# 0xPabloxx/3d-pointcloud-orientation-estimation

Hardware: AMD Instinct MI355X
Metric: clouds/sec fwd+bwd, pointnet_pp_vonMises N=1024 (higher is better)
Workload: dtype f32; 1 GPU; configs[1]: models/pointnet_pp_vonMises.py single-peak KL, N=1024, batch=32 per GPU, fwd+loss+bwd+allreduce+Adam, random-init weights (seed 42), device-side centre sampling; per_gpu_batch=32, global_batch=32, points=1024, parallelism=single, launch=hipGraph(fwd+loss+bwd) + eager all-reduce/Adam (the update clears the gradients)

## Files before the change

3d-pointcloud-orientation-estimation_amd/csrc/dw_kernels.hip:

```cpp
#include "gemm_smallm.h"
#include "launch.h"
#include "split_prims.h"

namespace pnpp {

template <int DZMODE, int A2MODE, int CT, int KT>
__global__ void __launch_bounds__(256)
dw_kernel(const AOperand dz, const AOperand a2, int M, int Nc, int Kp, int tilesC, int tilesK, int rows_per_split,
          int kp_pad, float *__restrict__ slab, int policy) {
    constexpr int U = 4;
    const int lane = threadIdx.x & 63, l31 = lane & 31, lh = lane >> 5;
    const int gw = blockIdx.x * 4 + (threadIdx.x >> 6);
    const int tiles = tilesC * tilesK;
    const int tile = gw % tiles, split = gw / tiles;
    const int r0 = min(M, split * rows_per_split);
    const int r1 = min(M, r0 + rows_per_split);
    const int c0 = (tile % tilesC) * 32 * CT, k0 = (tile / tilesC) * 32 * KT;

    ChanConst cc[CT], ck[KT];
#pragma unroll
    for (int i = 0; i < CT; ++i) cc[i] = load_chan_const<DZMODE>(dz, c0 + i * 32 + l31, Nc);
#pragma unroll
    for (int j = 0; j < KT; ++j) ck[j] = load_chan_const<A2MODE>(a2, k0 + j * 32 + l31, Kp);

    f32x16 acc[CT][KT];
#pragma unroll
    for (int i = 0; i < CT; ++i)
#pragma unroll
        for (int j = 0; j < KT; ++j)
#pragma unroll
            for (int r = 0; r < 16; ++r) acc[i][j][r] = 0.f;

// ... 171 lines not shown
        for (int e = 0; e < 4; ++e) d1[e] += (double)s1[e], d2[e] += (double)s2[e];
    }
    if (slab == nullptr) return;
#pragma unroll
    for (int e = 0; e < 4; ++e) {
        gred[(rl * 2 + 0) * C + c4 + e] = d1[e];
        gred[(rl * 2 + 1) * C + c4 + e] = d2[e];
    }
    __syncthreads();
    for (int f = threadIdx.x; f < 2 * C; f += 256) {
        const int which = f / C, c = f - which * C;
        double t = 0.0;
        for (int w = 0; w < RPP; ++w) t += gred[(w * 2 + which) * C + c];
        sp_store(slab + ((size_t)blockIdx.x * 2 + which) * C + c, t, (policy & ST_STAT_SLABS) != 0);
    }
}

bool delayed_layer0_ok(int C) {
    return C >= 32 && C <= 512 && (C & (C - 1)) == 0;
}

int launch_gather_rel_stats(const float *P, const AOperand &geo, const float *W0, int ldw, int M, int C, float *z,
                            double *slab, int *nslab, hipStream_t st) {
    PNPP_REQUIRE(delayed_layer0_ok(C) && geo.mode == A_GATHER, PNPP_ERR_ARG, "gather_rel_stats: unsupported width %d", C);
    const int rpp = 256 / (C / 4);
    int rpb = 64;
    while (rpb < 4 * rpp || cdiv(M, rpb) > kMaxStatBlocks) rpb *= 2;
    const int grid = cdiv(M, rpb);
    if (nslab) *nslab = grid;
    ProfScope ps(st, "gather_rel_stats_kernel M=%d C=%d grid=%d", M, C, grid);
    hipLaunchKernelGGL(gather_rel_stats_kernel, dim3(grid), dim3(256), (size_t)rpp * 2 * C * sizeof(double), st, P, geo.xyz,
                       geo.new_xyz, geo.idx, W0, ldw, geo.N, geo.S, geo.K, M, C, rpb, z, slab, store_policy());
    PNPP_CHECK_LAUNCH("gather_rel_stats");
    return PNPP_OK;
}

constexpr int SCW = 8;
constexpr int SCWIN = 1024;
template <int NCH>
__global__ void __launch_bounds__(SCW * 64)
scatter_dz_kernel(const AOperand dz, const AOperand geo, int Mc, int C, int total, float *__restrict__ G,
                  float *__restrict__ wslab) {
    constexpr int UB = NCH == 1 ? 8 : 4;
    __shared__ int hl[SCW][SCWIN];
    __shared__ float wred[SCW][NCH * 128][3];
    const int lane = threadIdx.x & 63, wv = threadIdx.x >> 6;
    const int N = geo.N;
    const int dst = min(blockIdx.x * SCW + wv, total - 1);
    const bool live = blockIdx.x * SCW + wv < total;
    const int b = dst / N, n = dst - b * N;
    const int32_t *ib = geo.idx + (size_t)b * Mc;
    const size_t row0 = (size_t)b * Mc;
    const float px = geo.xyz[(size_t)dst * 3], py = geo.xyz[(size_t)dst * 3 + 1], pz = geo.xyz[(size_t)dst * 3 + 2];
    const float *cb = geo.new_xyz + (size_t)b * geo.S * 3;
    float2 cg[NCH], cmu[NCH], cis[NCH], c1[NCH], c2[NCH], acc[NCH], ax[NCH], ay[NCH], az[NCH];
    int cc[NCH];
#pragma unroll
    for (int j = 0; j < NCH; ++j) {
        cc[j] = min(j * 128 + 2 * lane, C - 2);
        cg[j] = make_float2(1.f, 1.f);
        cmu[j] = cis[j] = c1[j] = c2[j] = acc[j] = ax[j] = ay[j] = az[j] = make_float2(0.f, 0.f);
        if (dz.mode == A_DZ) {
            const float *p = dz.cst + cc[j];
            cg[j] = *reinterpret_cast<const float2 *>(p), cmu[j] = *reinterpret_cast<const float2 *>(p + dz.C);
            cis[j] = *reinterpret_cast<const float2 *>(p + 2 * dz.C), c1[j] = *reinterpret_cast<const float2 *>(p + 3 * dz.C);
            c2[j] = *reinterpret_cast<const float2 *>(p + 4 * dz.C);
// ... 253 lines not shown
    if (!(M > 32 && M <= 4096 && cdiv(M, 32) <= kMaxStatBlocks && dz.mode == A_PLAIN && (dz.lda & 3) == 0 && ((uintptr_t)dz.a & 15) == 0))
        return false;
    if (!(Nc >= 128 && Kp >= 128 && Kd % 4 == 0 && !Win.trans && (E.mode == E_STORE || E.mode == E_MASK_STATS))) return false;
    if (!(a2.mode == A_PLAIN || a2.mode == A_BNRELU || a2.mode == A_CONCAT)) return false;
    if (a2.mode != A_CONCAT && ((a2.lda & 3) != 0 || ((uintptr_t)a2.a & 15) != 0)) return false;
    if (kp_pad != cdiv(Kp, 64) * 64 || nsplit < 1) return false;
    BOperand W = Win;
    if (W.rows <= 0 || W.rows > Kd) W.rows = Kd;
    const int g1x = cdiv(Nout, 32), g1y = cdiv(M, 32), g1 = g1x * g1y;
    const int tc = cdiv(Nc, 128), tk = cdiv(Kp, 128);
    int rps = cdiv(M, nsplit);
    rps = (rps + 7) & ~7;
    const dim3 grid(g1 + tc * tk * nsplit);
    if (nslab) *nslab = g1y;
    ProfScope ps(st, "da_dw_kernel<E%d,A%d> M=%d | dA N=%d K=%d grid=%d | dW N=%d K=%d split=%d grid=%d", E.mode, a2.mode, M, Nout, Kd, g1,
                 Nc, Kp, nsplit, tc * tk * nsplit);
#define PNPP_DADW(EM, AM) \
    hipLaunchKernelGGL((da_dw_kernel<EM, AM>), grid, dim3(256), 0, st, dz, W, M, Nout, Kd, E, g1x, g1, a2, Nc, Kp, tc, tk, rps, kp_pad, slab)
    if (E.mode == E_STORE) {
        if (a2.mode == A_PLAIN) PNPP_DADW(E_STORE, A_PLAIN);
        else if (a2.mode == A_BNRELU) PNPP_DADW(E_STORE, A_BNRELU);
        else PNPP_DADW(E_STORE, A_CONCAT);
    } else {
        if (a2.mode == A_PLAIN) PNPP_DADW(E_MASK_STATS, A_PLAIN);
        else if (a2.mode == A_BNRELU) PNPP_DADW(E_MASK_STATS, A_BNRELU);
        else PNPP_DADW(E_MASK_STATS, A_CONCAT);
    }
#undef PNPP_DADW
    check_launch("da_dw", rc);
    return true;
}

}
```

3d-pointcloud-orientation-estimation_amd/csrc/kernels.h:

```cpp
#pragma once
#include "common.h"

namespace pnpp {

int launch_knn(const float *new_xyz, const float *xyz, int B, int S, int N, int k, int32_t *idx, hipStream_t st,
               const int32_t *lengths = nullptr);
int launch_knn_centres(const float *xyz, const int32_t *centre, int B, int S, int N, int k, int32_t *idx, float *out_a,
                       float *out_b, hipStream_t st, const int32_t *lengths = nullptr);
int launch_knn_pair(const float *xyz, int B, int N, const int32_t *centre1, int S1, int k1, int32_t *idx1, float *a1, float *b1,
                    const int32_t *centre2, int S2, int k2, int32_t *idx2, float *a2, float *b2, double *mom, hipStream_t st,
                    const int32_t *lengths = nullptr);
int knn_pair_moment_partials(int B, int S1, int N);
size_t knn_pair_moment_doubles(int B, int S1, int N);
int launch_gather_centres(const float *xyz, const int32_t *centre, int B, int N, int S, float *out_a, float *out_b, hipStream_t st);
int launch_scatter_rows_bwd(const float *dout, const int32_t *idx, int B, int N, int C, int M, float *dpoints, hipStream_t st);

enum AMode {
    A_PLAIN = 0,
    A_BNRELU = 1,
    A_GATHER = 2,
    A_CONCAT = 3,
    A_DZ = 4,
    A_DZ_POOL = 5
};
// ... 75 lines not shown
struct PoolTail {
    const float *pool_ext = nullptr;
    float *pool_out = nullptr;
    int32_t *pool_arg = nullptr;
    float *origin_a = nullptr, *origin_b = nullptr;
    int G = 0, norigin = 0;
};
struct DzSide { const AOperand *dz = nullptr; int M = 0; float *out = nullptr; };
struct SlabReduceArgs {
    const float *slab;
    int nsplit, Nc, kp_pad, Kvalid, perm_D;
    float *out;
    int ldo;
};

int launch_gemm(const AOperand &A, const BOperand &B, int M, int Nout, int Kd, const Epilogue &E, int *nslab,
                hipStream_t st, int *dw_slabs = nullptr);
bool mid_tiles_on();
bool try_launch_ws(const AOperand &A, const BOperand &B, int M, int Nout, int Kd, const Epilogue &E, int *nslab, hipStream_t st, int *rc,
                   int *dw_slabs);

int matmul_precision();
void set_matmul_precision(int bf16);
bool try_launch_ws_bf16(const AOperand &A, const BOperand &B, int M, int Nout, int Kd, const Epilogue &E, int *nslab, hipStream_t st,
                        int *rc, int *dw_slabs);

int launch_dw(const AOperand &dz, int Nc, const AOperand &a2, int Kp, int M, float *slab, int nsplit, int kp_pad,
              hipStream_t st);
int launch_dz_materialize(const AOperand &dz, int M, int C, float *out, hipStream_t st);
void dw_plan(int M, int Nc, int Kp, int *nsplit, int *kp_pad);
bool delayed_layer0_ok(int C);
int launch_gather_rel_stats(const float *P, const AOperand &geo, const float *W0, int ldw, int M, int C, float *z,
                            double *slab, int *nslab, hipStream_t st);
int scatter_dz_splits(int rows);
int launch_scatter_dz(const AOperand &dz, const AOperand &geo, int B, int Mc, int C, float *G, float *wslab, hipStream_t st);
int dw_xyz_splits(int M);
int launch_dw_xyz(const AOperand &dz, int Nc, const AOperand &a2, int M, float *slab, hipStream_t st);
bool try_launch_fc_dx_dw(const float *dz, const float *w, const float *x, int M, int N, int K, float *dx, float *dw, hipStream_t st,
                         int *rc);
bool try_launch_da_dw(const AOperand &dz, const BOperand &W, int M, int Nout, int Kd, const Epilogue &E, int *nslab, const AOperand &a2,
                      int Kp, float *slab, int *nsplit, int *kp_pad, hipStream_t st, int *rc, float *dw_direct = nullptr, int dw_ld = 0);
bool try_launch_mid_gemm(const AOperand &A, const BOperand &B, int M, int Nout, int Kd, const Epilogue &E, int *nslab, hipStream_t st,
                         int *rc);
bool mid_gemm_pools(const AOperand &A, int M, int Nout, int Kd);
bool try_launch_wsf(const AOperand &A, const BOperand &B, int M, int Nout, int Kd, const Epilogue &E, int *nslab, hipStream_t st, int *rc);
bool wsf_applies(const AOperand &A, const BOperand &B, int M, int Nout, int Kd, const Epilogue &E);
int split_products();
void set_split_products(int on);
int store_policy();
void set_store_policy(int mask);
bool try_launch_wsf3(const AOperand &A, const BOperand &B, int M, int Nout, int Kd, const Epilogue &E, int *nslab, hipStream_t st, int *rc);
bool try_launch_wsd3(const AOperand &A, const BOperand &B, int M, int Nout, int Kd, const Epilogue &E, int *nslab, hipStream_t st, int *rc,
                     int *dw_slabs);
int wsd3_timeouts();
bool try_launch_wsp(const AOperand &A, const BOperand &B, int M, int Nout, int Kd, const Epilogue &E, int *nslab, hipStream_t st, int *rc,
                    int *dw_slabs);
bool try_launch_wsq(const AOperand &A, const BOperand &B, int M, int Nout, int Kd, const Epilogue &E, int *nslab, hipStream_t st, int *rc,
                    int *dw_slabs);
bool try_launch_wsx(const AOperand &dz, const BOperand &W, int M, int C1, int C0, const AOperand &geo, const float *W0, int ldw0,
                    const float *scale0, const float *shift0, float *dwslab, double *stat, int *workers_out, hipStream_t st, int *rc);
size_t wsx_stat_doubles();
bool xyz0_applies(int M, int D, int K, int group_all, int L, const int *C);
size_t xyz0_moment_doubles();
int launch_rel_moments(const AOperand &geo, int M, double *mom, int *nmom, hipStream_t st);
int launch_wsf0(const AOperand &geo, int M, const BOperand &W0, const double *mom, int nmom, const BnLayer &bn0, const BnHyper &h,
                const BOperand &W1, const Epilogue &E, int *nslab, hipStream_t st);
// ... 62 lines not shown
```

3d-pointcloud-orientation-estimation_amd/csrc/sa_api.hip:

```cpp
#include "launch.h"

namespace pnpp {

struct SaGeom {
    int M, G, maxC;
    int Cin[PNPP_MAX_LAYERS];
    int Kd[PNPP_MAX_LAYERS];
};

static int sa_geom(const pnpp_sa_desc *d, SaGeom *g) {
    PNPP_REQUIRE(d, PNPP_ERR_ARG, "sa: null descriptor");
    PNPP_REQUIRE(d->B > 0 && d->N > 0 && d->S > 0 && d->K > 0 && d->D >= 0, PNPP_ERR_ARG,
                 "sa: bad geometry B=%d N=%d S=%d K=%d D=%d", d->B, d->N, d->S, d->K, d->D);
    PNPP_REQUIRE(d->L >= 1 && d->L <= PNPP_MAX_LAYERS, PNPP_ERR_ARG, "sa: unsupported layer count %d", d->L);
    if (d->group_all) PNPP_REQUIRE(d->S == 1 && d->K == d->N, PNPP_ERR_ARG, "sa: group_all needs S == 1 and K == N");
    PNPP_REQUIRE((long long)d->B * d->S * d->K < (1ll << 31), PNPP_ERR_ARG, "sa: B*S*K overflows int32");
    g->M = d->B * d->S * d->K;
    g->G = d->B * d->S;
    g->maxC = 0;
    for (int l = 0; l < d->L; ++l) {
        PNPP_REQUIRE(d->C[l] > 0 && d->C[l] % 32 == 0, PNPP_ERR_ARG,
                     "sa: mlp channel %d (=%d) must be a positive multiple of 32 for the MFMA path", l, d->C[l]);
        g->maxC = d->C[l] > g->maxC ? d->C[l] : g->maxC;
        g->Cin[l] = l == 0 ? d->D + 3 : d->C[l - 1];
// ... 190 lines not shown
    sa_level_bind(L, a->saved, a->scratch, a->xyz, a->points, a->conv_w, a->bn_w, st);
    L->hyper = BnHyper{d->momentum, d->eps, d->training ? 1 : 0};
    return PNPP_OK;
}

static int sa_fwd_group(const SaLevel &L, const pnpp_sa_fwd_args *a) {
    const pnpp_sa_desc *d = L.d;
    const SaSaved &sv = L.sv;
    if (d->group_all) return PNPP_OK;
    PNPP_REQUIRE(d->S <= d->N, PNPP_ERR_RANGE, "sa_forward: npoint=%d > N=%d", d->S, d->N);
    if (a->neighbour_idx == sv.idx) return PNPP_OK;
    if (!a->neighbour_idx)
        return launch_knn_centres(a->xyz, a->centre_idx, d->B, d->S, d->N, d->K, sv.idx, a->new_xyz, sv.new_xyz, L.st);
    PNPP_TRY(launch_gather_centres(a->xyz, a->centre_idx, d->B, d->N, d->S, a->new_xyz, sv.new_xyz, L.st));
    hipError_t e = hipMemcpyAsync(sv.idx, a->neighbour_idx, (size_t)L.g.M * sizeof(int32_t), hipMemcpyDeviceToDevice, L.st);
    PNPP_REQUIRE(e == hipSuccess, PNPP_ERR_LAUNCH, "sa_forward: neighbour copy failed: %s", hipGetErrorString(e));
    return PNPP_OK;
}

static int sa_fwd_finalize(const SaLevel &L, int l, int nslab, const PoolTail *tail = nullptr) {
    StatsView V;
    if (L.d->training) PNPP_TRY(stats_exchange(L.sc.slab, nslab, L.d->C[l], L.count(), L.st, &V));
    return launch_bn_finalize_fwd(V, L.count(), L.bn[l], L.hyper, L.st, tail);
}

static int sa_fwd_gemm(const SaLevel &L, int l, const AOperand &A, const BOperand &W, const Epilogue &E, const double *mom, int nmom, int *ns) {
    if (L.xyz0 && l == 1)
        return launch_wsf0(L.layer0_operand(), L.g.M, L.weight(0, 0), mom, nmom, L.bn[0], L.hyper, L.weight(1, 0), E, ns, L.st);
    return launch_gemm(A, W, L.g.M, L.d->C[l], L.g.Kd[l], E, ns, L.st);
}

static int sa_fwd_delayed0(const SaLevel &L, const AOperand &geo) {
    const pnpp_sa_desc *d = L.d;
    AOperand F;
    F.a = L.points, F.lda = d->D;
    BOperand Wf = L.w0_features();
    Wf.trans = 1, Wf.rows = d->D;
    int nslab = 0;
    PNPP_TRY(launch_gemm(F, Wf, d->B * d->N, d->C[0], d->D, store_to(L.sc.src, d->C[0]), nullptr, L.st));
    PNPP_TRY(launch_gather_rel_stats(L.sc.src, geo, L.conv_w[0], L.g.Cin[0], L.g.M, d->C[0], L.sv.z[0], d->training ? L.sc.slab : nullptr,
                                     &nslab, L.st));
    return sa_fwd_finalize(L, 0, nslab);
}

static int sa_forward_impl(const pnpp_sa_desc *d, const pnpp_sa_fwd_args *a, hipStream_t st) {
    SaLevel L;
    PNPP_TRY(sa_level_fwd(d, a, st, &L));
    const SaGeom &g = L.g;
    const SaSaved &sv = L.sv;
    const SaScratch &sc = L.sc;
    PNPP_TRY(sa_fwd_group(L, a));
    const int Lm = d->L - 1;
    bool pooled = false;
    int nmom = 0;
    const double *mom = sc.mom;
    for (int l = 0; l < d->L; ++l) {
        if (L.xyz0 && l == 0) {
            if (!d->training) PNPP_TRY(sa_fwd_finalize(L, 0, 0));
            else if (a->neighbour_idx == sv.idx && L.pair_moments) mom = sv.mom, nmom = knn_pair_moment_partials(d->B, d->S, d->N);
            else PNPP_TRY(launch_rel_moments(L.layer0_operand(), g.M, sc.mom, &nmom, st));
            continue;
        }
        const AOperand A = L.input_of(l);
        if (l == 0 && L.delayed) {
            PNPP_TRY(sa_fwd_delayed0(L, A));
            continue;
// ... 331 lines not shown
```

3d-pointcloud-orientation-estimation_amd/csrc/split_prims.h:

```cpp
#pragma once
#include <type_traits>

#include "common.h"

namespace pnpp {
namespace {

typedef __bf16 bf16x8 __attribute__((ext_vector_type(8)));
typedef __bf16 bf16x2v __attribute__((ext_vector_type(2)));
typedef float f32x2v __attribute__((ext_vector_type(2)));
typedef short s16x4 __attribute__((ext_vector_type(4)));

__device__ __forceinline__ unsigned sp_pk(float lo, float hi) {
    const f32x2v v = {lo, hi};
    return __builtin_bit_cast(unsigned, __builtin_convertvector(v, bf16x2v));
}
__device__ __forceinline__ float sp_lo(unsigned p) { return __uint_as_float(p << 16); }
__device__ __forceinline__ float sp_hi(unsigned p) { return __uint_as_float(p & 0xffff0000u); }
__device__ __forceinline__ void sp_split2(float v0, float v1, unsigned &h, unsigned &m, unsigned &l) {
    h = sp_pk(v0, v1);
    float r0 = v0 - sp_lo(h), r1 = v1 - sp_hi(h);
    m = sp_pk(r0, r1);
    r0 -= sp_lo(m), r1 -= sp_hi(m);
    l = sp_pk(r0, r1);
// ... 16 lines not shown
    const s16x4 v = __builtin_amdgcn_ds_read_tr16_b64_v4i16((__attribute__((address_space(3))) s16x4 *)(p));
    return __builtin_bit_cast(uint2, v);
}
__device__ __forceinline__ constexpr int sp_swz_row(int r) { return (((r >> 1) & 1) << 2) | ((r >> 2) & 3); }

__device__ __forceinline__ __amdgpu_buffer_rsrc_t sp_buf_rsrc_n(const void *base, unsigned records) {
    return __builtin_amdgcn_make_buffer_rsrc(const_cast<void *>(base), (short)0, records, 0x00020000);
}
__device__ __forceinline__ __amdgpu_buffer_rsrc_t sp_buf_rsrc(const void *base) { return sp_buf_rsrc_n(base, 0xfffffffe); }
__device__ __forceinline__ __amdgpu_buffer_rsrc_t sp_buf_rsrc_null(const void *base) { return sp_buf_rsrc_n(base, 0); }
__device__ __forceinline__ f32x4 sp_buf_load4(__amdgpu_buffer_rsrc_t r, unsigned lane_off, unsigned s_off) {
    return __builtin_bit_cast(f32x4, __builtin_amdgcn_raw_buffer_load_b128(r, (int)lane_off, (int)s_off, 0));
}
__device__ __forceinline__ float sp_buf_load1(__amdgpu_buffer_rsrc_t r, unsigned lane_off, unsigned s_off) {
    return __builtin_bit_cast(float, __builtin_amdgcn_raw_buffer_load_b32(r, (int)lane_off, (int)s_off, 0));
}

template <typename F>
__device__ __forceinline__ void sp_with_policy(bool wt, F &&f) {
    if (wt) f(std::true_type{});
    else f(std::false_type{});
}
template <typename T>
__device__ __forceinline__ void sp_store(T *p, T v, bool wt) {
    static_assert(sizeof(T) == 4 || sizeof(T) == 8, "one dword or two per lane");
    typedef __attribute__((address_space(1))) T gT;
    if (wt) __hip_atomic_store((gT *)p, v, __ATOMIC_RELAXED, __HIP_MEMORY_SCOPE_AGENT);
    else *p = v;
}
__device__ __forceinline__ void sp_buf_store1(float v, __amdgpu_buffer_rsrc_t r, unsigned lane_off, unsigned s_off, bool wt) {
    if (wt) __builtin_amdgcn_raw_buffer_store_b32(__builtin_bit_cast(unsigned, v), r, (int)lane_off, (int)s_off, 16);
    else __builtin_amdgcn_raw_buffer_store_b32(__builtin_bit_cast(unsigned, v), r, (int)lane_off, (int)s_off, 0);
}

}
}
```

3d-pointcloud-orientation-estimation_amd/pnpp_hip/_lib.py:

```python
from __future__ import annotations

import ctypes as C
import os

HERE = os.path.dirname(os.path.abspath(__file__))
LIB_PATH = os.path.join(HERE, "libpnpp_hip.so")

PNPP_MAX_LAYERS = 4
PNPP_OK, PNPP_ERR_ARG, PNPP_ERR_RANGE, PNPP_ERR_LAUNCH, PNPP_ERR_WORKSPACE = 0, -1, -2, -3, -4
NORM_NONE, NORM_BATCH, NORM_LAYER = 0, 1, 2

_fp = C.c_void_p


class SaDesc(C.Structure):
    _fields_ = [("B", C.c_int), ("N", C.c_int), ("S", C.c_int), ("K", C.c_int), ("D", C.c_int), ("L", C.c_int),
                ("C", C.c_int * PNPP_MAX_LAYERS), ("group_all", C.c_int), ("training", C.c_int),
                ("eps", C.c_float), ("momentum", C.c_float)]


_PL = _fp * PNPP_MAX_LAYERS


class SaFwdArgs(C.Structure):
# ... 210 lines not shown
    "pnpp_orient_eval": (_i, [_fp, _fp, _fp, _i, _i, _fp, _fp, _fp, _fp, _i, _fp, _i, _fp, _fp, C.c_int64, _fp, _fp, _fp, _fp]),
    "pnpp_log_softmax": (_i, [_fp, _i, _i, _fp, _fp]),
    "pnpp_log_softmax_bwd": (_i, [_fp, _fp, _i, _i, _fp, _fp]),
    "pnpp_linear_log_softmax": (_i, [_fp, _fp, _fp, _i, _i, _i, _fp, _fp]),
    "pnpp_nll_loss": (_i, [_fp, _fp, _i, _i, _fp, _fp, _i, _fp]),
    "pnpp_nll_loss_bwd": (_i, [_fp, _fp, _i, _i, _fp, _fp]),
    "pnpp_l2_normalize": (_i, [_fp, _i, _i, _f, _fp, _fp]),
    "pnpp_l2_normalize_bwd": (_i, [_fp, _fp, _i, _i, _f, _fp, _fp]),
    "pnpp_mse": (_i, [_fp, _fp, _sz, _fp, _fp, _fp]),
    "pnpp_mse_rows": (_i, [_fp, _fp, _i, _i, _fp, _fp, _fp]),
    "pnpp_orth_loss": (_i, [_fp, _fp, _i, _i, _fp, _fp, _fp, _fp]),
    "pnpp_proj_probs": (_i, [_fp, _fp, _i, _i, _fp, _fp]),
    "pnpp_proj_probs_bwd": (_i, [_fp, _fp, _fp, _i, _i, _fp, _fp]),
    "pnpp_linear_smallk": (_i, [_fp, _fp, _fp, _i, _i, _i, _fp, _fp]),
    "pnpp_attention_fwd": (_i, [_fp, _i, _i, _i, _i, _i, _fp, _f, _fp, _fp, _fp]),
    "pnpp_attention_dropout_mask": (_i, [_u64, _u64, _i, _i, _i, _f, _fp, _fp, _fp]),
    "pnpp_attention_dropout_mask_dev": (_i, [_u64, _fp, _u64, _i, _i, _i, _f, _fp, _fp, _fp]),
    "pnpp_add_layernorm": (_i, [_fp, _fp, _fp, _fp, _i, _i, _f, _fp, _fp]),
    "pnpp_mean_points": (_i, [_fp, _i, _i, _i, _fp, _fp]),
    "pnpp_linear_smallk_bwd_scratch_bytes": (_sz, [_i, _i]),
    "pnpp_linear_smallk_bwd": (_i, [_fp, _fp, _i, _i, _i, _fp, _fp, _fp, _fp]),
    "pnpp_attention_bwd": (_i, [_fp, _fp, _fp, _fp, _i, _i, _i, _i, _i, _fp, _fp, _f, _fp, _fp, _fp]),
    "pnpp_add_layernorm_bwd_scratch_bytes": (_sz, [_i, _i]),
    "pnpp_add_layernorm_bwd": (_i, [_fp, _fp, _fp, _fp, _i, _i, _f, _fp, _fp, _fp, _fp]),
    "pnpp_mean_points_bwd": (_i, [_fp, _i, _i, _i, _fp, _fp]),
    "pnpp_set_matmul_precision": (_i, [_i]),
    "pnpp_set_stats_exchange": (_i, [STATS_EXCHANGE_FN, C.c_void_p, C.c_void_p, _sz]),
    "pnpp_stats_exchange_enabled": (_i, []),
    "pnpp_get_matmul_precision": (_i, []),
    "pnpp_set_split_products": (_i, [_i]),
    "pnpp_get_split_products": (_i, []),
    "pnpp_set_store_policy": (_i, [_i]),
    "pnpp_get_store_policy": (_i, []),
    "pnpp_adam_step": (_i, [_fp, _fp, _fp, _fp, _sz, _i, _f, _f, _f, _f, _f, _fp]),
    "pnpp_adam_step_zero": (_i, [_fp, _fp, _fp, _fp, _sz, _i, _f, _f, _f, _f, _f, _fp]),
    "pnpp_adam_step_dev": (_i, [_fp, _fp, _fp, _fp, _sz, _fp, _f, _f, _f, _f, _f, _i, _fp]),
    "pnpp_adam_step_clip": (_i, [_fp, _fp, _fp, _fp, _sz, _i, _f, _f, _f, _f, _f, _fp, _f, _i, _fp]),
    "pnpp_adam_step_dev_clip": (_i, [_fp, _fp, _fp, _fp, _sz, _fp, _f, _f, _f, _f, _f, _fp, _f, _i, _fp]),
    "pnpp_sumsq": (_i, [_fp, _sz, _fp, _fp, _sz, _fp]),
    "pnpp_adamw_step": (_i, [C.POINTER(OptimDesc), _fp, _fp, _fp, _fp, _fp, _sz, _fp, _fp, _fp]),
    "pnpp_lr_factor": (_i, [C.POINTER(OptimDesc), _u64, C.POINTER(C.c_double)]),
    "pnpp_pn_pool_saved_bytes": (_sz, [C.POINTER(PnPoolDesc)]),
    "pnpp_pn_pool_scratch_bytes": (_sz, [C.POINTER(PnPoolDesc)]),
    "pnpp_pn_pool_forward": (_i, [C.POINTER(PnPoolDesc), C.POINTER(PnPoolFwdArgs), _fp]),
    "pnpp_pn_pool_backward": (_i, [C.POINTER(PnPoolDesc), C.POINTER(PnPoolBwdArgs), _fp]),
    "pnpp_pn_pool_saved_route": (_fp, [C.POINTER(PnPoolDesc), _fp]),
    "pnpp_pn_pool_saved_zsel": (_fp, [C.POINTER(PnPoolDesc), _fp]),
    "pnpp_pn_pool_saved_ypre": (_fp, [C.POINTER(PnPoolDesc), _fp]),
    "pnpp_fc_recompute_output": (_i, [C.POINTER(FcDesc), _fp, _fp, _fp, _fp]),
    "pnpp_pn_transform": (_i, [_fp, C.c_int64, C.c_int64, C.c_int64, _fp, _i, _i, _i, _i, _i, _fp, _fp]),
    "pnpp_pn_transform_bwd": (_i, [_fp, C.c_int64, C.c_int64, C.c_int64, _fp, _fp, _i, _i, _i, _i, _i, _fp, _fp, _fp]),
    "pnpp_pn_regularizer": (_i, [_fp, _i, _i, _fp, _fp, _fp]),
    "pnpp_pn_regularizer_bwd": (_i, [_fp, _fp, _fp, _i, _i, _fp, _fp]),
    "pnpp_pn_add_identity": (_i, [_fp, _i, _i, _fp, _fp]),
    "pnpp_pn_concat": (_i, [_fp, _fp, _i, _i, _i, _i, _fp, _fp]),
    "pnpp_pn_concat_bwd": (_i, [_fp, _i, _i, _i, _i, _fp, _fp, _fp]),
    "pnpp_pn_bn_relu": (_i, [_fp, _i, _i, _fp, _fp, _fp, _fp, _fp, _i, _f, _f, _fp, _fp, _fp, _fp]),
    "pnpp_pn_bn_relu_bwd": (_i, [_fp, _fp, _fp, _i, _i, _fp, _fp, _fp, _i, _fp, _fp, _fp, _fp]),
    "pnpp_pn_offsets": (_i, [_fp, _i, _i, _fp, _fp, _fp]),
    "pnpp_pn_pool_saved_bytes_ragged": (_sz, [C.POINTER(PnPoolDesc), _i]),
    "pnpp_pn_pool_scratch_bytes_ragged": (_sz, [C.POINTER(PnPoolDesc), _i]),
    "pnpp_pn_pool_forward_ragged": (_i, [C.POINTER(PnPoolDesc), C.POINTER(PnPoolFwdArgs), _fp, _i, _fp]),
    "pnpp_pn_pool_backward_ragged": (_i, [C.POINTER(PnPoolDesc), C.POINTER(PnPoolBwdArgs), _fp, _i, _fp]),
    "pnpp_pn_transform_ragged": (_i, [_fp, _i, C.c_int64, C.c_int64, C.c_int64, _fp, _fp, _i, _i, _i, _i, _i, _fp, _fp]),
    "pnpp_pn_transform_bwd_ragged": (_i, [_fp, _i, C.c_int64, C.c_int64, C.c_int64, _fp, _fp, _fp, _i, _i, _i, _i, _i, _fp, _fp, _fp]),
    "pnpp_pn_concat_ragged": (_i, [_fp, _fp, _i, _fp, _i, _i, _i, _i, _fp, _fp]),
# ... 44 lines not shown
```

3d-pointcloud-orientation-estimation_amd/pnpp_hip/ops.py:

```python
from __future__ import annotations

import ctypes as C
import os
from typing import Optional, Sequence, Tuple

import torch

from . import _lib as L
from .lengths import fps_starts, packed_lengths, ragged_lengths


def _stream() -> int:
    return torch.cuda.current_stream().cuda_stream


def _need_gpu(t: torch.Tensor, name: str) -> None:
    if not isinstance(t, torch.Tensor):
        raise TypeError(f"{name} must be a torch.Tensor")
    if not t.is_cuda:
        raise RuntimeError(f"{name} is on '{t.device}': the pnpp HIP operators run on an AMD GPU only "
                           "(no CPU fallback exists in this package)")


def _f32(t: torch.Tensor, name: str) -> torch.Tensor:
# ... 83 lines not shown
        returned.append(fresh)
    return dests, returned


def set_matmul_precision(mode: str) -> None:
    if mode not in ("f32", "bf16"):
        raise ValueError(f"matmul precision must be 'f32' or 'bf16', got {mode!r}")
    L.check(L.lib().pnpp_set_matmul_precision(1 if mode == "bf16" else 0))


def get_matmul_precision() -> str:
    return "bf16" if L.lib().pnpp_get_matmul_precision() else "f32"


def set_float32_products(mode: str) -> None:
    if mode not in ("split", "mfma"):
        raise ValueError(f"float32 products must be 'split' or 'mfma', got {mode!r}")
    L.check(L.lib().pnpp_set_split_products(1 if mode == "split" else 0))


def get_float32_products() -> str:
    return "split" if L.lib().pnpp_get_split_products() else "mfma"


STORE_DW_SLABS, STORE_STAT_SLABS, STORE_STREAMS = 1, 2, 4


def set_store_policy(mask: int) -> None:
    L.check(L.lib().pnpp_set_store_policy(int(mask)))


def get_store_policy() -> int:
    return L.lib().pnpp_get_store_policy()


def square_distance(src: torch.Tensor, dst: torch.Tensor) -> torch.Tensor:
    src, dst = _f32(src, "src"), _f32(dst, "dst")
    B, S, _ = src.shape
    N = dst.shape[1]
    out = torch.empty(B, S, N, device=src.device, dtype=torch.float32)
    L.check(L.lib().pnpp_square_distance(src.data_ptr(), dst.data_ptr(), B, S, N, out.data_ptr(), _stream()))
    return out


def knn(new_xyz: torch.Tensor, xyz: torch.Tensor, k: int, lengths=None) -> torch.Tensor:
    new_xyz, xyz = _f32(new_xyz, "new_xyz"), _f32(xyz, "xyz")
    B, S, _ = new_xyz.shape
    N = xyz.shape[1]
    idx = torch.empty(B, S, k, device=xyz.device, dtype=torch.int32)
    if lengths is not None:
        lengths = ragged_lengths(lengths, B, N, xyz.device, minimum=k)
        L.check(L.lib().pnpp_knn_ragged(new_xyz.data_ptr(), xyz.data_ptr(), B, S, N, lengths.data_ptr(), int(k), idx.data_ptr(), _stream()))
        return idx
    L.check(L.lib().pnpp_knn(new_xyz.data_ptr(), xyz.data_ptr(), B, S, N, int(k), idx.data_ptr(), _stream()))
    return idx


def estimate_normals(xyz: torch.Tensor, k: int, mode: int = L.NORMALS_NONE, ref: Optional[torch.Tensor] = None, lengths=None,
                     stride: int = 3, curvature: bool = False, neighbours: bool = False):
    xyz = _f32(xyz, "xyz")
    if xyz.dim() != 3 or xyz.shape[2] != 3:
        raise ValueError(f"xyz must be (B, N, 3), got {tuple(xyz.shape)}")
    B, N, _ = xyz.shape
    if ref is not None:
        ref = _f32(ref, "ref")
        if tuple(ref.shape) != (B, 3):
# ... 1498 lines not shown
```

include/pnpp_hip.h:

```cpp
#ifndef PNPP_HIP_H
#define PNPP_HIP_H

#include <stddef.h>
#include <stdint.h>

#ifdef __cplusplus
extern "C" {
#endif

typedef enum {
    PNPP_OK = 0,
    PNPP_ERR_ARG = -1,
    PNPP_ERR_RANGE = -2,
    PNPP_ERR_LAUNCH = -3,
    PNPP_ERR_WORKSPACE = -4
} pnpp_status;

const char *pnpp_last_error(void);
int pnpp_abi_version(void);

int pnpp_profile_enable(int on);
int pnpp_profile_report(char *buf_host, size_t buflen);


// ... 224 lines not shown
int pnpp_orth_loss(const float *a, const float *b, int B, int C, float *loss, float *da, float *db, void *stream);
int pnpp_proj_probs(const float *vec, const float *dirs, int B, int D, float *probs, void *stream);
int pnpp_proj_probs_bwd(const float *vec, const float *dirs, const float *dprobs, int B, int D, float *dvec, void *stream);

int pnpp_linear_smallk(const float *x, const float *w, const float *b, int M, int K, int N, float *y, void *stream);
int pnpp_attention_fwd(const float *qkv, int B, int N, int n_valid, int H, int head_dim, const uint32_t *mask, float p,
                       float *out, float *lse, void *stream);
int pnpp_attention_dropout_mask(uint64_t seed, uint64_t stream_id, int B, int N, int H, float p, uint32_t *mask,
                                uint32_t *maskT, void *stream);
int pnpp_attention_dropout_mask_dev(uint64_t seed, uint64_t *stream_id_dev, uint64_t offset, int B, int N, int H, float p,
                                    uint32_t *mask, uint32_t *maskT, void *stream);
int pnpp_add_layernorm(const float *x, const float *r, const float *w, const float *b, int M, int E, float eps, float *y,
                       void *stream);
int pnpp_mean_points(const float *x, int B, int N, int E, float *y, void *stream);
size_t pnpp_linear_smallk_bwd_scratch_bytes(int M, int N);
int pnpp_linear_smallk_bwd(const float *x, const float *dy, int M, int K, int N, float *dw, float *db, void *scratch,
                           void *stream);
int pnpp_attention_bwd(const float *qkv, const float *out, const float *d_out, const float *lse, int B, int N, int n_valid, int H,
                       int head_dim, const uint32_t *mask, const uint32_t *maskT, float p, float *dqkv, float *dsum,
                       void *stream);
size_t pnpp_add_layernorm_bwd_scratch_bytes(int M, int E);
int pnpp_add_layernorm_bwd(const float *x, const float *r, const float *w, const float *dy, int M, int E, float eps,
                           float *du, float *dwb, void *scratch, void *stream);
int pnpp_mean_points_bwd(const float *dy, int B, int N, int E, float *dx, void *stream);

int pnpp_set_matmul_precision(int bf16_operands);
int pnpp_get_matmul_precision(void);

int pnpp_set_split_products(int on);
int pnpp_get_split_products(void);

int pnpp_set_store_policy(int mask);
int pnpp_get_store_policy(void);
int pnpp_debug_wsd3_timeouts(void);

typedef int (*pnpp_stats_exchange_fn)(double *buf, size_t n_doubles, void *stream, void *user);
int pnpp_set_stats_exchange(pnpp_stats_exchange_fn fn, void *user, double *buf, size_t buf_doubles);
int pnpp_stats_exchange_enabled(void);

typedef struct {
    int B, N;
    int K, C;
    int relu;
    int training;
    float eps, momentum;
} pnpp_pn_pool_desc;

typedef struct {
    const float *a;
    const float *w, *b;
    const float *gamma, *beta;
    float *rm, *rv;
    int64_t *nbt;
    float *out;
    void *saved;
    void *scratch;
} pnpp_pn_pool_fwd_args;

typedef struct {
    const float *a, *w, *gamma;
    const float *dout;
    const void *saved;
    void *scratch;
    float *da;
    float *dw, *db, *dgamma, *dbeta;
} pnpp_pn_pool_bwd_args;
// ... 233 lines not shown
```

Baseline: 61050 clouds/s.

## Fuse per-point feature GEMM into delayed layer-0 gather/stats kernel

Adds a fused kernel for the delayed layer-0 path. Each block computes the per-point feature projection P = F·W0 for its batch and channel slice in LDS using MFMA, then gathers neighbour rows, adds the relative-xyz term and accumulates the BN statistics in the same launch. Before, a separate GEMM wrote P to global memory and the stats kernel read it back. The fused form removes one launch and that global round trip, but every share block recomputes P for its whole cloud, and the large LDS footprint may lower occupancy. It is on by default (form=1) when the shape checks pass.

```diff
diff --git a/3d-pointcloud-orientation-estimation_amd/csrc/dw_kernels.hip b/3d-pointcloud-orientation-estimation_amd/csrc/dw_kernels.hip
--- a/3d-pointcloud-orientation-estimation_amd/csrc/dw_kernels.hip
+++ b/3d-pointcloud-orientation-estimation_amd/csrc/dw_kernels.hip
@@ -1,3 +1,5 @@
+#include <algorithm>
+
 #include "gemm_smallm.h"
 #include "launch.h"
 #include "split_prims.h"
@@ -235,6 +237,224 @@
     hipLaunchKernelGGL(gather_rel_stats_kernel, dim3(grid), dim3(256), (size_t)rpp * 2 * C * sizeof(double), st, P, geo.xyz,
                        geo.new_xyz, geo.idx, W0, ldw, geo.N, geo.S, geo.K, M, C, rpb, z, slab, store_policy());
     PNPP_CHECK_LAUNCH("gather_rel_stats");
+    return PNPP_OK;
+}
+
+constexpr int D0_SL = 32;
+constexpr int D0_PP = D0_SL + 4;
+constexpr int D0_ROWS = 256 / (D0_SL / 4);
+constexpr size_t kDelayed0LdsMax = 80 * 1024;
+constexpr int kDelayed0MaxRows = 2048;
+
+static size_t delayed0_lds_bytes(int N, int S, int D, int rps) {
+    const size_t npad = (size_t)cdiv(N, 32) * 32;
+    return sizeof(float) * ((size_t)4 * 32 * APITCH + npad * D0_PP + 4 * (size_t)N + 4 * (size_t)S + (size_t)D0_SL * (D + 1) + (size_t)rps);
+}
+
+static int delayed0_shares(int B, int SK, int C, int *rows_per_share) {
+    int shares = cdiv(256, B * (C / D0_SL));
+    shares = std::min(shares, std::max(1, SK / (4 * D0_ROWS)));
+    shares = std::max(shares, cdiv(SK, kDelayed0MaxRows));
+    const int rps = cdiv(SK, shares);
+    *rows_per_share = rps;
+    return cdiv(SK, rps);
+}
+
+bool delayed0_fused_ok(int B, int N, int S, int K, int D, int C) {
+    if (!(B >= 1 && N >= 1 && S >= 1 && K >= 1 && (long long)S * K < (1 << 24) && D >= 32 && D % 32 == 0 && C % D0_SL == 0 && delayed_layer0_ok(C))) return false;
+    int rps = 0;
+    const int shares = delayed0_shares(B, S * K, C, &rps);
+    return (long long)B * shares <= kMaxStatBlocks && delayed0_lds_bytes(N, S, D, rps) <= kDelayed0LdsMax;
+}
+
+__global__ void __launch_bounds__(256)
+gather_rel_stats_fused_kernel(const float *__restrict__ F, const float *__restrict__ xyz, const float *__restrict__ new_xyz,
+                              const int32_t *__restrict__ idx, const float *__restrict__ W0, int ldw, int B, int N, int S, int K,
+                              int D, int C, int shares, int rps, float *__restrict__ z, double *__restrict__ slab, int policy) {
+    extern __shared__ __attribute__((aligned(16))) float d0lds[];
+    const int tid = threadIdx.x, lane = tid & 63, wave = tid >> 6, l31 = lane & 31, lh = lane >> 5;
+    const int nsl = C / D0_SL, per = nsl * shares;
+    const int q = blockIdx.x >> 3;
+    const int b = (blockIdx.x & 7) + 8 * (q / per);
+    if (b >= B) return;
+    const int sub = q % per, c0 = (sub % nsl) * D0_SL, share = sub / nsl;
+    const int SK = S * K, r0 = share * rps, r1 = min(SK, r0 + rps);
+    const int ntiles = (N + 31) >> 5, nch = D >> 5, WP = D + 1;
+    float *As = d0lds + wave * 32 * APITCH;
+    float *Pl = d0lds + 4 * 32 * APITCH;
+    float4 *Xl = reinterpret_cast<float4 *>(Pl + ntiles * 32 * D0_PP);
+    float4 *Cl = Xl + N;
+    float *Wl = reinterpret_cast<float *>(Cl + S);
+    int *Il = reinterpret_cast<int *>(Wl + D0_SL * WP);
+    const float *Fb = F + (size_t)b * N * D;
+    const int32_t *ib = idx + (size_t)b * SK;
+
+    float4 na[2][4];
+    auto fetch_a = [&](float4(&d)[4], int t, int c) {
+#pragma unroll
+        for (int i = 0; i < 4; ++i) {
+            const int row = min(t * 32 + (lane >> 3) + 8 * i, N - 1);
+            d[i] = *reinterpret_cast<const float4 *>(Fb + (size_t)row * D + c * KC + 4 * (lane & 7));
+        }
+    };
+    auto fetch_a2 = [&](int t) {
+        fetch_a(na[0], t, 0);
+        if (nch > 1) fetch_a(na[1], t, 1);
+    };
+    if (wave < ntiles) fetch_a2(wave);
+    const int rl = tid >> 3, c4 = (tid & 7) * 4;
+    const int i0 = ib[min(r0 + tid, r1 - 1)], i1 = ib[min(r0 + 256 + tid, r1 - 1)];
+    float wx[4], wy[4], wz[4];
+#pragma unroll
+    for (int e = 0; e < 4; ++e) {
+        const float *w = W0 + (size_t)(c0 + c4 + e) * ldw;
+        wx[e] = w[0], wy[e] = w[1], wz[e] = w[2];
+    }
+    const float *xp = xyz + ((size_t)b * N + min(tid, N - 1)) * 3, *cp = new_xyz + ((size_t)b * S + min(tid, S - 1)) * 3;
+    const float x0 = xp[0], x1 = xp[1], x2 = xp[2], q0 = cp[0], q1 = cp[1], q2 = cp[2];
+    {
+        int wr = tid / D, wk = tid - wr * D;
+        const int dq = 256 / D, dm = 256 - dq * D;
+        auto w_batch = [&](auto nb) {
+            float t[nb()];
+            int o[nb()];
+#pragma unroll
+            for (int u = 0; u < nb(); ++u) {
+                t[u] = W0[(size_t)(c0 + wr) * ldw + 3 + wk];
+                o[u] = wr * WP + wk;
+                wr += dq, wk += dm;
+                if (wk >= D) wk -= D, ++wr;
+            }
+#pragma unroll
+            for (int u = 0; u < nb(); ++u) Wl[o[u]] = t[u];
+        };
+        int e0 = 0;
+        for (; e0 + 4096 <= D0_SL * D; e0 += 4096) w_batch(mode_c<16>{});
+        for (; e0 < D0_SL * D; e0 += 1024) w_batch(mode_c<4>{});
+    }
+    if (tid < N) Xl[tid] = make_float4(x0, x1, x2, 0.f);
+    if (tid < S) Cl[tid] = make_float4(q0, q1, q2, 0.f);
+    if (r0 + tid < r1) Il[tid] = i0;
+    if (r0 + 256 + tid < r1) Il[256 + tid] = i1;
+    for (int i = r0 + 512 + tid; i < r1; i += 256) Il[i - r0] = ib[i];
+    for (int i = tid + 256; i < N; i += 256) {
+        const float *x = xyz + ((size_t)b * N + i) * 3;
+        Xl[i] = make_float4(x[0], x[1], x[2], 0.f);
+    }
+    for (int i = tid + 256; i < S; i += 256) {
+        const float *c = new_xyz + ((size_t)b * S + i) * 3;
+        Cl[i] = make_float4(c[0], c[1], c[2], 0.f);
+    }
+    __syncthreads();
+
+    for (int t = wave; t < ntiles; t += 4) {
+        f32x16 acc4[4];
+#pragma unroll
+        for (int i = 0; i < 4; ++i)
+#pragma unroll
+            for (int r = 0; r < 16; ++r) acc4[i][r] = 0.f;
+        if (t != wave) fetch_a2(t);
+        auto chunk = [&](f32x16 &acc, float4(&d)[4], int c) {
+#pragma unroll
+            for (int i = 0; i < 4; ++i) {
+                const int o = ((lane >> 3) + 8 * i) * APITCH + 4 * (lane & 7);
+                As[o] = d[i].x, As[o + 1] = d[i].y, As[o + 2] = d[i].z, As[o + 3] = d[i].w;
+            }
+            if (c + 2 < nch) fetch_a(d, t, c + 2);
+            const float *wk = Wl + l31 * WP + c * KC + lh;
+#pragma unroll
+            for (int s2 = 0; s2 < KC / 2; ++s2)
+                acc = __builtin_amdgcn_mfma_f32_32x32x2f32(As[l31 * APITCH + 2 * s2 + lh], wk[2 * s2], acc, 0, 0, 0);
+        };
+        for (int c = 0; c < nch; c += 4) {
+            chunk(acc4[0], na[0], c);
+            if (c + 1 < nch) chunk(acc4[1], na[1], c + 1);
+            if (c + 2 < nch) chunk(acc4[2], na[0], c + 2);
+            if (c + 3 < nch) chunk(acc4[3], na[1], c + 3);
+        }
+#pragma unroll
+        for (int r = 0; r < 16; ++r)
+            Pl[(t * 32 + (r & 3) + 8 * (r >> 2) + 4 * lh) * D0_PP + l31] = (acc4[0][r] + acc4[1][r]) + (acc4[2][r] + acc4[3][r]);
+    }
+    __syncthreads();
+
+    double d1[4] = {0.0, 0.0, 0.0, 0.0}, d2[4] = {0.0, 0.0, 0.0, 0.0};
+    float *zc = z + (size_t)b * SK * C;
+    const int Ro = 1024 / C, ro = (rl / Ro) * 4 * Ro + rl % Ro;
+    const float rcpK = 1.f / (float)K;
+    const __amdgpu_buffer_rsrc_t zr = sp_buf_rsrc(zc);
+    sp_with_policy((policy & ST_STREAMS) != 0, [&](auto wt) {
+    for (int rb = r0 + ro; rb - ro < r1; rb += 4 * D0_ROWS) {
+        int jc[4];
+#pragma unroll
+        for (int u = 0; u < 4; ++u) jc[u] = Il[min(rb + u * Ro, r1 - 1) - r0];
+        float4 p[4];
+        float rx[4], ry[4], rz[4], ok[4];
+#pragma unroll
+        for (int u = 0; u < 4; ++u) {
+            const int r = rb + u * Ro;
+            ok[u] = r < r1 ? 1.f : 0.f;
+            p[u] = *reinterpret_cast<const float4 *>(Pl + jc[u] * D0_PP + c4);
+            const int rc = min(r, r1 - 1);
+            int g = (int)((float)rc * rcpK);
+            g += (int)((g + 1) * K <= rc) - (int)(g * K > rc);
+            const float4 x = Xl[jc[u]], c = Cl[g];
+            rx[u] = __fsub_rn(x.x, c.x), ry[u] = __fsub_rn(x.y, c.y), rz[u] = __fsub_rn(x.z, c.z);
+        }
+        float s1[4] = {0.f, 0.f, 0.f, 0.f}, s2[4] = {0.f, 0.f, 0.f, 0.f};
+#pragma unroll
+        for (int u = 0; u < 4; ++u) {
+            float v[4] = {p[u].x, p[u].y, p[u].z, p[u].w};
+#pragma unroll
+            for (int e = 0; e < 4; ++e) {
+                v[e] = fmaf(rz[u], wz[e], fmaf(ry[u], wy[e], fmaf(rx[u], wx[e], v[e])));
+                const float m = v[e] * ok[u];
+                s1[e] += m, s2[e] = fmaf(m, m, s2[e]);
+            }
+            const int r = rb + u * Ro;
+            if (r < r1) sp_buf_store4(f32x4{v[0], v[1], v[2], v[3]}, zr, (unsigned)(((size_t)r * C + c0 + c4) * sizeof(float)), 0, wt());
+        }
+#pragma unroll
+        for (int e = 0; e < 4; ++e) d1[e] += (double)s1[e], d2[e] += (double)s2[e];
+    }
+    });
+    if (slab == nullptr) return;
+    double *gred = reinterpret_cast<double *>(d0lds);
+#pragma unroll
+    for (int e = 0; e < 4; ++e) {
+        gred[(rl * 2 + 0) * D0_SL + c4 + e] = d1[e];
+        gred[(rl * 2 + 1) * D0_SL + c4 + e] = d2[e];
+    }
+    __syncthreads();
+    if (tid < 2 * D0_SL) {
+        const int which = tid / D0_SL, c = tid - which * D0_SL;
+        double t = 0.0;
+#pragma unroll
+        for (int w = 0; w < D0_ROWS; ++w) t += gred[(w * 2 + which) * D0_SL + c];
+        sp_store(slab + ((size_t)(b * shares + share) * 2 + which) * C + c0 + c, t, (policy & ST_STAT_SLABS) != 0);
+    }
+}
+
+static int g_delayed0_form = 1;
+int delayed0_form() { return g_delayed0_form; }
+void set_delayed0_form(int form) { g_delayed0_form = form; }
+
+int launch_gather_rel_stats_fused(const float *F, const AOperand &geo, const float *W0, int ldw, int B, int D, int C, float *z,
+                                  double *slab, int *nslab, hipStream_t st) {
+    PNPP_REQUIRE(geo.mode == A_GATHER && delayed0_fused_ok(B, geo.N, geo.S, geo.K, D, C), PNPP_ERR_ARG,
+                 "gather_rel_stats (fused): unsupported shape N=%d S=%d D=%d C=%d", geo.N, geo.S, D, C);
+    const int SK = geo.S * geo.K;
+    int rps = 0;
+    const int shares = delayed0_shares(B, SK, C, &rps);
+    PNPP_REQUIRE((size_t)SK * C * sizeof(float) < 0xfffffff0u, PNPP_ERR_RANGE, "gather_rel_stats (fused): a cloud's rows exceed a buffer's 4 GB");
+    const int grid = 8 * (C / D0_SL) * shares * cdiv(B, 8);
+    if (nslab) *nslab = B * shares;
+    const size_t lds = delayed0_lds_bytes(geo.N, geo.S, D, rps);
+    grant_lds<gather_rel_stats_fused_kernel>(lds);
+    ProfScope ps(st, "gather_rel_stats_kernel M=%d C=%d grid=%d +P D=%d", B * SK, C, grid, D);
+    hipLaunchKernelGGL(gather_rel_stats_fused_kernel, dim3(grid), dim3(256), lds, st, F, geo.xyz, geo.new_xyz, geo.idx, W0, ldw, B,
+                       geo.N, geo.S, geo.K, D, C, shares, rps, z, slab, store_policy());
+    PNPP_CHECK_LAUNCH("gather_rel_stats (fused)");
     return PNPP_OK;
 }
 
@@ -554,3 +774,14 @@
 }
 
 }
+
+extern "C" int pnpp_set_delayed0_form(int form) {
+    if (form != 0 && form != 1) {
+        pnpp::set_error("pnpp_set_delayed0_form: form %d is neither 0 (two launches) nor 1 (fused)", form);
+        return PNPP_ERR_ARG;
+    }
+    pnpp::set_delayed0_form(form);
+    return PNPP_OK;
+}
+extern "C" int pnpp_get_delayed0_form(void) { return pnpp::delayed0_form(); }
+extern "C" int pnpp_delayed0_fused_ok(int B, int N, int S, int K, int D, int C) { return pnpp::delayed0_fused_ok(B, N, S, K, D, C) ? 1 : 0; }
diff --git a/3d-pointcloud-orientation-estimation_amd/csrc/kernels.h b/3d-pointcloud-orientation-estimation_amd/csrc/kernels.h
--- a/3d-pointcloud-orientation-estimation_amd/csrc/kernels.h
+++ b/3d-pointcloud-orientation-estimation_amd/csrc/kernels.h
@@ -131,6 +131,11 @@
 bool delayed_layer0_ok(int C);
 int launch_gather_rel_stats(const float *P, const AOperand &geo, const float *W0, int ldw, int M, int C, float *z,
                             double *slab, int *nslab, hipStream_t st);
+bool delayed0_fused_ok(int B, int N, int S, int K, int D, int C);
+int delayed0_form();
+void set_delayed0_form(int form);
+int launch_gather_rel_stats_fused(const float *F, const AOperand &geo, const float *W0, int ldw, int B, int D, int C, float *z,
+                                  double *slab, int *nslab, hipStream_t st);
 int scatter_dz_splits(int rows);
 int launch_scatter_dz(const AOperand &dz, const AOperand &geo, int B, int Mc, int C, float *G, float *wslab, hipStream_t st);
 int dw_xyz_splits(int M);
diff --git a/3d-pointcloud-orientation-estimation_amd/csrc/sa_api.hip b/3d-pointcloud-orientation-estimation_amd/csrc/sa_api.hip
--- a/3d-pointcloud-orientation-estimation_amd/csrc/sa_api.hip
+++ b/3d-pointcloud-orientation-estimation_amd/csrc/sa_api.hip
@@ -246,6 +246,12 @@
 
 static int sa_fwd_delayed0(const SaLevel &L, const AOperand &geo) {
     const pnpp_sa_desc *d = L.d;
+    if (delayed0_form() == 1 && delayed0_fused_ok(d->B, d->N, d->S, d->K, d->D, d->C[0])) {
+        int nslab = 0;
+        PNPP_TRY(launch_gather_rel_stats_fused(L.points, geo, L.conv_w[0], L.g.Cin[0], d->B, d->D, d->C[0], L.sv.z[0],
+                                               d->training ? L.sc.slab : nullptr, &nslab, L.st));
+        return sa_fwd_finalize(L, 0, nslab);
+    }
     AOperand F;
     F.a = L.points, F.lda = d->D;
     BOperand Wf = L.w0_features();
diff --git a/3d-pointcloud-orientation-estimation_amd/csrc/split_prims.h b/3d-pointcloud-orientation-estimation_amd/csrc/split_prims.h
--- a/3d-pointcloud-orientation-estimation_amd/csrc/split_prims.h
+++ b/3d-pointcloud-orientation-estimation_amd/csrc/split_prims.h
@@ -72,6 +72,11 @@
     if (wt) __builtin_amdgcn_raw_buffer_store_b32(__builtin_bit_cast(unsigned, v), r, (int)lane_off, (int)s_off, 16);
     else __builtin_amdgcn_raw_buffer_store_b32(__builtin_bit_cast(unsigned, v), r, (int)lane_off, (int)s_off, 0);
 }
+__device__ __forceinline__ void sp_buf_store4(f32x4 v, __amdgpu_buffer_rsrc_t r, unsigned lane_off, unsigned s_off, bool wt) {
+    typedef __attribute__((ext_vector_type(4))) unsigned u32x4;
+    if (wt) __builtin_amdgcn_raw_buffer_store_b128(__builtin_bit_cast(u32x4, v), r, (int)lane_off, (int)s_off, 16);
+    else __builtin_amdgcn_raw_buffer_store_b128(__builtin_bit_cast(u32x4, v), r, (int)lane_off, (int)s_off, 0);
+}
 
 }
 }
diff --git a/3d-pointcloud-orientation-estimation_amd/pnpp_hip/_lib.py b/3d-pointcloud-orientation-estimation_amd/pnpp_hip/_lib.py
--- a/3d-pointcloud-orientation-estimation_amd/pnpp_hip/_lib.py
+++ b/3d-pointcloud-orientation-estimation_amd/pnpp_hip/_lib.py
@@ -266,6 +266,9 @@
     "pnpp_get_split_products": (_i, []),
     "pnpp_set_store_policy": (_i, [_i]),
     "pnpp_get_store_policy": (_i, []),
+    "pnpp_set_delayed0_form": (_i, [_i]),
+    "pnpp_get_delayed0_form": (_i, []),
+    "pnpp_delayed0_fused_ok": (_i, [_i, _i, _i, _i, _i, _i]),
     "pnpp_adam_step": (_i, [_fp, _fp, _fp, _fp, _sz, _i, _f, _f, _f, _f, _f, _fp]),
     "pnpp_adam_step_zero": (_i, [_fp, _fp, _fp, _fp, _sz, _i, _f, _f, _f, _f, _f, _fp]),
     "pnpp_adam_step_dev": (_i, [_fp, _fp, _fp, _fp, _sz, _fp, _f, _f, _f, _f, _f, _i, _fp]),
diff --git a/3d-pointcloud-orientation-estimation_amd/pnpp_hip/ops.py b/3d-pointcloud-orientation-estimation_amd/pnpp_hip/ops.py
--- a/3d-pointcloud-orientation-estimation_amd/pnpp_hip/ops.py
+++ b/3d-pointcloud-orientation-estimation_amd/pnpp_hip/ops.py
@@ -139,6 +139,18 @@
 
 def get_store_policy() -> int:
     return L.lib().pnpp_get_store_policy()
+
+
+def set_delayed0_form(form: int) -> None:
+    L.check(L.lib().pnpp_set_delayed0_form(int(form)))
+
+
+def get_delayed0_form() -> int:
+    return L.lib().pnpp_get_delayed0_form()
+
+
+def delayed0_fused_ok(B: int, N: int, S: int, K: int, D: int, C0: int) -> bool:
+    return bool(L.lib().pnpp_delayed0_fused_ok(int(B), int(N), int(S), int(K), int(D), int(C0)))
 
 
 def square_distance(src: torch.Tensor, dst: torch.Tensor) -> torch.Tensor:
diff --git a/include/pnpp_hip.h b/include/pnpp_hip.h
--- a/include/pnpp_hip.h
+++ b/include/pnpp_hip.h
@@ -280,6 +280,9 @@
 
 int pnpp_set_store_policy(int mask);
 int pnpp_get_store_policy(void);
+int pnpp_set_delayed0_form(int form);
+int pnpp_get_delayed0_form(void);
+int pnpp_delayed0_fused_ok(int B, int N, int S, int K, int D, int C);
 int pnpp_debug_wsd3_timeouts(void);
 
 typedef int (*pnpp_stats_exchange_fn)(double *buf, size_t n_doubles, void *stream, void *user);
```

Result: no change. 61600 clouds/s, median of 6 (+0.9%).
